# edouardoyallon/acco

Measured on AMD Instinct MI355X. Metric: tokens/s, higher is better.
Workload: dtype bf16; 1 GPU; model=llama-1b, method=acco, global_batch=8, seq_len=1024, parallelism=acco-dp1, comm_buckets=8, params=1076168704, ckpt=False

## Files before the change

acco_amd/ops/csrc/attention_bwd.hip:

```cpp

#include "attention_common.h"
#include "kernels.h"

namespace {

using namespace attn;

template <int D, int QW>
__global__ __launch_bounds__(256)
void attn_bwd_dq_kernel(const u16* __restrict__ q, const u16* __restrict__ k,
                        const u16* __restrict__ v, const u16* __restrict__ dO,
                        const float* __restrict__ lse,
                        const float* __restrict__ delta,
                        u16* __restrict__ dq,
                        int S, int H, int Hkv, float scale, int window) {
  constexpr int KS = D / 32;
  constexpr int DT = D / 16;
  constexpr int KROW = D + 8;
  constexpr int M2 = QW / 16;
  constexpr int QT = 4 * QW;
  const int qt = blockIdx.x, bh = blockIdx.y;
  const int b = bh / H, h = bh % H, hkv = h / (H / Hkv);
  const int wave = threadIdx.x >> 6, lane = threadIdx.x & 63;
  const int lg = lane >> 4, lc = lane & 15;

  extern __shared__ __attribute__((aligned(16))) u16 smem[];
  using L = BwdDqLds<D, 4>;
  u16* kT_lds = smem + L::k_t;
  u16* k_row = smem + L::k_row;
  u16* v_row = smem + L::v_row;
  u16* ds_lds = smem + L::ds + wave * 16 * LST;

  const long long qs = (long long)H * D, ks = (long long)Hkv * D;
  const int q0 = qt * QT + wave * QW;
  const u16* Qp = q + ((long long)b * S + q0) * qs + (long long)h * D;
  const u16* dOp = dO + ((long long)b * S + q0) * qs + (long long)h * D;
  const u16* Kb = k + (long long)b * S * ks + (long long)hkv * D;
  const u16* Vb = v + (long long)b * S * ks + (long long)hkv * D;

  short8 qf[M2][KS], dof[M2][KS];
  float lse_c[M2], delta_c[M2];
#pragma unroll
  for (int m = 0; m < M2; ++m) {
#pragma unroll
    for (int s = 0; s < KS; ++s) {
      qf[m][s] = *reinterpret_cast<const short8*>(
          Qp + (long long)(m * 16 + lc) * qs + s * 32 + lg * 8);
      dof[m][s] = *reinterpret_cast<const short8*>(
          dOp + (long long)(m * 16 + lc) * qs + s * 32 + lg * 8);
    }
    lse_c[m] = lse[(long long)bh * S + q0 + m * 16 + lc];
    delta_c[m] = delta[(long long)bh * S + q0 + m * 16 + lc];
  }

// ... 55 lines not shown
        for (int t = 0; t < DT; ++t) {
          short8 kb = *reinterpret_cast<const short8*>(
              kT_lds + (t * 16 + lc) * LST + s * 32 + lg * 8);
          acc_dq[m][t] = MFMA(dsa, kb, acc_dq[m][t]);
        }
      }
    }
  }

  u16* dQp = dq + ((long long)b * S + q0) * qs + (long long)h * D;
#pragma unroll
  for (int m = 0; m < M2; ++m)
#pragma unroll
    for (int r = 0; r < 4; ++r)
#pragma unroll
      for (int t = 0; t < DT; ++t)
        dQp[(long long)(m * 16 + lg * 4 + r) * qs + t * 16 + lc] =
            f32_to_bf16(acc_dq[m][t][r]);
}

template <int D, int QW>
__global__ __launch_bounds__(256)
void attn_bwd_dkv_kernel(const u16* __restrict__ q, const u16* __restrict__ k,
                         const u16* __restrict__ v, const u16* __restrict__ dO,
                         const float* __restrict__ lse,
                         const float* __restrict__ delta,
                         u16* __restrict__ dk, u16* __restrict__ dv,
                         int S, int H, int Hkv, float scale, int window) {
  constexpr int KS = D / 32;
  constexpr int DT = D / 16;
  constexpr int KROW = D + 8;
  constexpr int M2 = QW / 16;
  constexpr int KB = 4 * QW;
  const int jb = blockIdx.x, bh = blockIdx.y;
  const int b = bh / H, h = bh % H, hkv = h / (H / Hkv);
  const int wave = threadIdx.x >> 6, lane = threadIdx.x & 63;
  const int lg = lane >> 4, lc = lane & 15;

  extern __shared__ __attribute__((aligned(16))) u16 smem[];
  using L = BwdDkvLds<D, 4>;
  u16* qT_lds = smem + L::q_t;
  u16* doT_lds = smem + L::do_t;
  u16* q_row = smem + L::q_row;
  u16* do_row = smem + L::do_row;
  u16* p_lds = smem + L::p + wave * 16 * LST;
  u16* ds_lds = smem + L::p + (4 + wave) * 16 * LST;

  const long long qs = (long long)H * D, ks = (long long)Hkv * D;
  const int kv0 = jb * KB + wave * QW;
  const u16* Kp = k + ((long long)b * S + kv0) * ks + (long long)hkv * D;
  const u16* Vp = v + ((long long)b * S + kv0) * ks + (long long)hkv * D;
  const u16* Qb = q + (long long)b * S * qs + (long long)h * D;
  const u16* dOb = dO + (long long)b * S * qs + (long long)h * D;

  short8 kTf[M2][KS], vTf[M2][KS];
#pragma unroll
  for (int m = 0; m < M2; ++m)
#pragma unroll
    for (int s = 0; s < KS; ++s) {
      kTf[m][s] = *reinterpret_cast<const short8*>(
          Kp + (long long)(m * 16 + lc) * ks + s * 32 + lg * 8);
      vTf[m][s] = *reinterpret_cast<const short8*>(
          Vp + (long long)(m * 16 + lc) * ks + s * 32 + lg * 8);
    }

  f32x4 acc_dk[M2][DT] = {}, acc_dv[M2][DT] = {};

// ... 71 lines not shown
  }

  u16* dKp = dk + ((long long)b * S + kv0) * qs + (long long)h * D;
  u16* dVp = dv + ((long long)b * S + kv0) * qs + (long long)h * D;
#pragma unroll
  for (int m = 0; m < M2; ++m)
#pragma unroll
    for (int r = 0; r < 4; ++r)
#pragma unroll
      for (int t = 0; t < DT; ++t) {
        dKp[(long long)(m * 16 + lg * 4 + r) * qs + t * 16 + lc] =
            f32_to_bf16(acc_dk[m][t][r]);
        dVp[(long long)(m * 16 + lg * 4 + r) * qs + t * 16 + lc] =
            f32_to_bf16(acc_dv[m][t][r]);
      }
}

}

extern "C" {

void acco_attn_bwd_dq(const void* q, const void* k, const void* v,
                      const void* dO, const float* lse, const float* delta,
                      void* dq, int B, int S, int H, int Hkv, int D,
                      float scale, int window, hipStream_t stream) {
  if (use_mfma32(S, D)) {
    acco_attn_bwd32_dq(q, k, v, dO, lse, delta, dq, B, S, H, Hkv, D, scale,
                       window, (long long)H * D, (long long)Hkv * D,
                       (long long)H * D, (long long)H * D, nullptr, nullptr,
                       stream);
    return;
  }
  const bool w = wide(S, D);
  dim3 grid(S / (w ? 128 : 64), B * H);
#define LQ(DD, QQ) hipLaunchKernelGGL((attn_bwd_dq_kernel<DD, QQ>), grid, \
    dim3(256), (BwdDqLds<DD, 4>::bytes), stream, (const u16*)q, \
    (const u16*)k, (const u16*)v, (const u16*)dO, lse, delta, (u16*)dq, S, H, \
    Hkv, scale, window)
  if (D == 64) { if (w) LQ(64, 32); else LQ(64, 16); }
  else         LQ(128, 16);
#undef LQ
}

void acco_attn_bwd_dkv(const void* q, const void* k, const void* v,
                       const void* dO, const float* lse, const float* delta,
                       void* dk, void* dv, int B, int S, int H, int Hkv,
                       int D, float scale, int window, hipStream_t stream) {
  if (use_mfma32(S, D)) {
    acco_attn_bwd32_dkv(q, k, v, dO, lse, delta, dk, dv, B, S, H, Hkv, D,
                        scale, window, (long long)H * D, (long long)Hkv * D,
                        (long long)H * D, stream);
    return;
  }
  const bool w = wide(S, D);
  dim3 grid(S / (w ? 128 : 64), B * H);
#define LK(DD, QQ) hipLaunchKernelGGL((attn_bwd_dkv_kernel<DD, QQ>), grid, \
    dim3(256), (BwdDkvLds<DD, 4>::bytes), stream, (const u16*)q, \
    (const u16*)k, (const u16*)v, (const u16*)dO, lse, delta, (u16*)dk, \
    (u16*)dv, S, H, Hkv, scale, window)
  if (D == 64) { if (w) LK(64, 32); else LK(64, 16); }
  else         LK(128, 16);
#undef LK
}

}
```

acco_amd/ops/csrc/attention_bwd32.hip:

```cpp

#include "attention_common.h"
#include "kernels.h"

namespace {

using namespace attn;

template <int D>
__global__ __launch_bounds__(512, D == 64 ? 4 : 2)
void attn_bwd32_dq_kernel(const u16* __restrict__ q, const u16* __restrict__ k,
                          const u16* __restrict__ v, const u16* __restrict__ dO,
                          const float* __restrict__ lse,
                          const float* __restrict__ delta,
                          u16* __restrict__ dq,
                          int S, int H, int Hkv, float scale, int window,
                          long long q_rs, long long kv_rs, long long do_rs,
                          long long dq_rs,
                          const float* __restrict__ rope_cos,
                          const float* __restrict__ rope_sin) {
  constexpr int KS = D / 16;
  constexpr int DT = D / 32;
  constexpr int KROW = D + 8;
  const int qt = blockIdx.x, bh = blockIdx.y;
  const int b = bh / H, h = bh % H, hkv = h / (H / Hkv);
  const int wave = threadIdx.x >> 6, lane = threadIdx.x & 63;
  const int lq = lane & 31, hi = lane >> 5;

  extern __shared__ __attribute__((aligned(16))) u16 smem[];
  using L = Bwd32DqLds<D>;
  u16* k_row = smem + L::k_row;
  u16* v_row = smem + L::v_row;
  u16* kT_lds = smem + L::k_t;

  const long long qs = q_rs, ks = kv_rs;
  const int q0 = qt * BT32 + wave * QW32;
  const u16* Qp = q + ((long long)b * S + q0) * qs + (long long)h * D;
  const u16* dOp = dO + ((long long)b * S + q0) * do_rs + (long long)h * D;
  const u16* Kb = k + (long long)b * S * ks + (long long)hkv * D;
  const u16* Vb = v + (long long)b * S * ks + (long long)hkv * D;

  short8 qf[KS], dof[KS];
#pragma unroll
  for (int s = 0; s < KS; ++s) {
    qf[s] = *reinterpret_cast<const short8*>(
        Qp + (long long)lq * qs + s * 16 + hi * 8);
    dof[s] = *reinterpret_cast<const short8*>(
        dOp + (long long)lq * do_rs + s * 16 + hi * 8);
  }
  const float lse2_c = lse[(long long)bh * S + q0 + lq] * 1.4426950408889634f;
  const float delta_s = delta[(long long)bh * S + q0 + lq] * scale;
  const float scale2 = scale * 1.4426950408889634f;

  f32x16 acc_dq[DT] = {};

  const int j_lo = kv_tile_lo(qt * BT32, window);
  const int j_hi = kv_tile_hi(qt * BT32, BT32);
// ... 61 lines not shown
      const float* sr = rope_sin + (long long)(q0 + qrow) * D + lq;
#pragma unroll
      for (int t = 0; t < DT / 2; ++t) {
        const float c = cr[t * 32], sn = sr[t * 32];
        const float g1 = bf16_to_f32(f32_to_bf16(acc_dq[t][r]));
        const float g2 = bf16_to_f32(f32_to_bf16(acc_dq[t + DT / 2][r]));
        acc_dq[t][r] = __fmaf_rn(g1, c, __fmul_rn(g2, sn));
        acc_dq[t + DT / 2][r] = __fmaf_rn(g2, c, -__fmul_rn(g1, sn));
      }
    }
  }
#pragma unroll
  for (int r = 0; r < 16; ++r) {
    const int qrow = c32_row(r, hi);
#pragma unroll
    for (int t = 0; t < DT; ++t)
      dQp[(long long)qrow * dq_rs + t * 32 + lq] = f32_to_bf16(acc_dq[t][r]);
  }
}

template <int D>
__global__ __launch_bounds__(512)
void attn_bwd32_dkv_kernel(const u16* __restrict__ q, const u16* __restrict__ k,
                           const u16* __restrict__ v,
                           const u16* __restrict__ dO,
                           const float* __restrict__ lse,
                           const float* __restrict__ delta,
                           u16* __restrict__ dk, u16* __restrict__ dv,
                           int S, int H, int Hkv, float scale, int window,
                           long long q_rs, long long kv_rs, long long do_rs) {
  constexpr int KS = D / 16;
  constexpr int DT = D / 32;
  constexpr int KROW = D + 8;
  const int jb = blockIdx.x, bh = blockIdx.y;
  const int b = bh / H, h = bh % H, hkv = h / (H / Hkv);
  const int wave = threadIdx.x >> 6, lane = threadIdx.x & 63;
  const int lq = lane & 31, hi = lane >> 5;

  extern __shared__ __attribute__((aligned(16))) u16 smem[];
  using L = Bwd32DkvLds<D>;
  u16* q_row = smem + L::q_row;
  u16* do_row = smem + L::do_row;
  u16* qT_lds = smem + L::q_t;
  u16* doT_lds = smem + L::do_t;

  const long long qs = q_rs, ks = kv_rs;
  const long long od = (long long)H * D;
  const int kv0 = jb * BT32 + wave * QW32;
  const u16* Kp = k + ((long long)b * S + kv0) * ks + (long long)hkv * D;
  const u16* Vp = v + ((long long)b * S + kv0) * ks + (long long)hkv * D;
  const u16* Qb = q + (long long)b * S * qs + (long long)h * D;
  const u16* dOb = dO + (long long)b * S * do_rs + (long long)h * D;

  constexpr bool KV_RES = (D == 64);
  short8 kTf[KV_RES ? KS : 1], vTf[KV_RES ? KS : 1];
  if constexpr (KV_RES) {
#pragma unroll
    for (int s = 0; s < KS; ++s) {
      kTf[s] = *reinterpret_cast<const short8*>(
          Kp + (long long)lq * ks + s * 16 + hi * 8);
      vTf[s] = *reinterpret_cast<const short8*>(
          Vp + (long long)lq * ks + s * 16 + hi * 8);
    }
  }

  f32x16 acc_dk[DT] = {}, acc_dv[DT] = {};

  const int qt_lo = q_tile_lo(jb * BT32);
  const int qt_hi = q_tile_hi(jb * BT32, BT32, S, window);
  const int kv_wave_min = kv0;

  const bool t_q = (threadIdx.x < 256);
  const int t_id = threadIdx.x & 255;
  const int t_d0 = (t_id % 32) * 2;
  const int t_kv8 = (t_id / 32) * 8;
  unsigned streg[8];
  static_assert(TILE * (D / 8) % 512 == 0, "rowmajor chunks");
  constexpr int RCH = TILE * (D / 8) / 512;
  uint4 rq[RCH], rdo[RCH];

  auto load_qtile = [&](int qt) {
    const u16* Qs = Qb + (long long)(qt * TILE) * qs;
    const u16* Ds = dOb + (long long)(qt * TILE) * do_rs;
    if (D == 64) {
      const u16* Ts = t_q ? Qs : Ds;
      const long long tstride = t_q ? qs : do_rs;
#pragma unroll
      for (int r = 0; r < 8; ++r)
        streg[r] = *reinterpret_cast<const unsigned*>(
            Ts + (long long)(t_kv8 + r) * tstride + t_d0);
    }
#pragma unroll
    for (int c = 0; c < RCH; ++c) {
      const int cc = threadIdx.x + c * 512;
      const int r = cc / (D / 8), dc = cc % (D / 8);
      rq[c] = *reinterpret_cast<const uint4*>(Qs + (long long)r * qs + dc * 8);
      rdo[c] = *reinterpret_cast<const uint4*>(Ds + (long long)r * do_rs + dc * 8);
    }
  };
  auto write_qtile = [&]() {
    if (D == 64) {
      uint4 lo, hi4;
      lo.x = (streg[0] & 0xffffu) | (streg[1] << 16);
      lo.y = (streg[2] & 0xffffu) | (streg[3] << 16);
      lo.z = (streg[4] & 0xffffu) | (streg[5] << 16);
      lo.w = (streg[6] & 0xffffu) | (streg[7] << 16);
      hi4.x = (streg[0] >> 16) | (streg[1] & 0xffff0000u);
      hi4.y = (streg[2] >> 16) | (streg[3] & 0xffff0000u);
      hi4.z = (streg[4] >> 16) | (streg[5] & 0xffff0000u);
      hi4.w = (streg[6] >> 16) | (streg[7] & 0xffff0000u);
      u16* dst = t_q ? qT_lds : doT_lds;
      *reinterpret_cast<uint4*>(dst + t_d0 * LST + t_kv8) = lo;
      *reinterpret_cast<uint4*>(dst + (t_d0 + 1) * LST + t_kv8) = hi4;
    }
#pragma unroll
    for (int c = 0; c < RCH; ++c) {
      const int cc = threadIdx.x + c * 512;
      const int r = cc / (D / 8), dc = cc % (D / 8);
      reinterpret_cast<uint4*>(q_row + r * KROW)[dc] = rq[c];
      reinterpret_cast<uint4*>(do_row + r * KROW)[dc] = rdo[c];
    }
  };

  auto stage_qtile_direct = [&](int qt) {
    const u16* Qs = Qb + (long long)(qt * TILE) * qs;
    const u16* Ds = dOb + (long long)(qt * TILE) * do_rs;
    stage_transposed<D, 512>(Qs, qs, qT_lds);
    stage_transposed<D, 512>(Ds, do_rs, doT_lds);
    stage_rowmajor<D, 512>(Qs, qs, q_row);
    stage_rowmajor<D, 512>(Ds, do_rs, do_row);
  };

  if constexpr (KV_RES) load_qtile(qt_lo);
  for (int qt = qt_lo; qt <= qt_hi; ++qt) {
    __syncthreads();
    if constexpr (KV_RES) {
      write_qtile();
    } else {
      stage_qtile_direct(qt);
    }
    __syncthreads();
    if constexpr (KV_RES)
      if (qt < qt_hi) load_qtile(qt + 1);
    if (qt * TILE + TILE - 1 < kv_wave_min) continue;

#pragma unroll
    for (int m32 = 0; m32 < 2; ++m32) {
      const float lse_l =
          lse[(long long)bh * S + qt * TILE + m32 * 32 + lq] * 1.4426950408889634f;
      const float del_l =
          delta[(long long)bh * S + qt * TILE + m32 * 32 + lq] * scale;

      f32x16 st = {}, dpt = {};
      __builtin_amdgcn_s_setprio(1);
      if constexpr (KV_RES) {
#pragma unroll
        for (int s = 0; s < KS; ++s) {
          short8 qfr = *reinterpret_cast<const short8*>(
              q_row + (m32 * 32 + lq) * KROW + s * 16 + hi * 8);
          short8 dofr = *reinterpret_cast<const short8*>(
              do_row + (m32 * 32 + lq) * KROW + s * 16 + hi * 8);
          st = MFMA32(qfr, kTf[s], st);
          dpt = MFMA32(dofr, vTf[s], dpt);
        }
      } else {
#pragma unroll 2
        for (int s = 0; s < KS; ++s) {
          short8 qfr = *reinterpret_cast<const short8*>(
              q_row + (m32 * 32 + lq) * KROW + s * 16 + hi * 8);
          short8 dofr = *reinterpret_cast<const short8*>(
              do_row + (m32 * 32 + lq) * KROW + s * 16 + hi * 8);
          short8 kf = *reinterpret_cast<const short8*>(
              Kp + (long long)lq * ks + s * 16 + hi * 8);
          short8 vf = *reinterpret_cast<const short8*>(
              Vp + (long long)lq * ks + s * 16 + hi * 8);
          st = MFMA32(qfr, kf, st);
          dpt = MFMA32(dofr, vf, dpt);
        }
      }
      __builtin_amdgcn_s_setprio(0);

      const int kv_g = kv0 + lq;
      const float scale2_ = scale * 1.4426950408889634f;
      const bool need_mask =
          (qt * TILE < kv0 + QW32 - 1) ||
          (window > 0 && kv0 + window <= qt * TILE + TILE - 1);
#pragma unroll
      for (int r = 0; r < 16; ++r) {
        const int rr = c32_row(r, hi);
        const float lse_q = __shfl(lse_l, rr, 64);
        const float del_q = __shfl(del_l, rr, 64);
        float x = st[r] * scale2_ - lse_q;
        if (need_mask) {
          const int q_g = qt * TILE + m32 * 32 + rr;
          x = attends(kv_g, q_g, window) ? x : -1e30f;
        }
        const float pval = __builtin_amdgcn_exp2f(x);
        st[r] = pval;
        dpt[r] = pval * __builtin_fmaf(dpt[r], scale, -del_q);
      }

      __builtin_amdgcn_s_setprio(1);
#pragma unroll
      for (int kk = 0; kk < 2; ++kk) {
        short8 pa = c_to_afrag(st, kk);
        short8 dsa = c_to_afrag(dpt, kk);
#pragma unroll
        for (int t = 0; t < DT; ++t) {
          short8 dob = *reinterpret_cast<const short8*>(
              doT_lds + (t * 32 + lq) * LST + m32 * 32 + kk * 16 + hi * 8);
          short8 qb = *reinterpret_cast<const short8*>(
              qT_lds + (t * 32 + lq) * LST + m32 * 32 + kk * 16 + hi * 8);
          acc_dv[t] = MFMA32(pa, dob, acc_dv[t]);
          acc_dk[t] = MFMA32(dsa, qb, acc_dk[t]);
        }
      }
      __builtin_amdgcn_s_setprio(0);
    }
  }

  u16* dKp = dk + ((long long)b * S + kv0) * od + (long long)h * D;
  u16* dVp = dv + ((long long)b * S + kv0) * od + (long long)h * D;
#pragma unroll
  for (int r = 0; r < 16; ++r) {
    const int krow = c32_row(r, hi);
#pragma unroll
    for (int t = 0; t < DT; ++t) {
      dKp[(long long)krow * od + t * 32 + lq] = f32_to_bf16(acc_dk[t][r]);
      dVp[(long long)krow * od + t * 32 + lq] = f32_to_bf16(acc_dv[t][r]);
    }
  }
}

}

extern "C" {

void acco_attn_bwd32_dq(const void* q, const void* k, const void* v,
                        const void* dO, const float* lse, const float* delta,
                        void* dq, int B, int S, int H, int Hkv, int D,
                        float scale, int window, long long q_rs,
                        long long kv_rs, long long do_rs, long long dq_rs,
                        const float* rope_cos, const float* rope_sin,
                        hipStream_t stream) {
  dim3 grid(S / BT32, B * H);
#define LQ(DD) hipLaunchKernelGGL(attn_bwd32_dq_kernel<DD>, grid, dim3(512), \
    Bwd32DqLds<DD>::bytes, stream, (const u16*)q, (const u16*)k, \
    (const u16*)v, (const u16*)dO, lse, delta, (u16*)dq, S, H, Hkv, scale, \
    window, q_rs, kv_rs, do_rs, dq_rs, rope_cos, rope_sin)
  if (D == 64) LQ(64); else LQ(128);
#undef LQ
}

void acco_attn_bwd32_dkv(const void* q, const void* k, const void* v,
                         const void* dO, const float* lse,
                         const float* delta, void* dk, void* dv, int B,
                         int S, int H, int Hkv, int D, float scale,
                         int window, long long q_rs, long long kv_rs,
                         long long do_rs, hipStream_t stream) {
  dim3 grid(S / BT32, B * H);
#define LK(DD) hipLaunchKernelGGL(attn_bwd32_dkv_kernel<DD>, grid, dim3(512), \
    Bwd32DkvLds<DD>::bytes, stream, (const u16*)q, (const u16*)k, \
    (const u16*)v, (const u16*)dO, lse, delta, (u16*)dk, (u16*)dv, S, H, Hkv, \
    scale, window, q_rs, kv_rs, do_rs)
  if (D == 64) LK(64); else LK(128);
#undef LK
}

}
```

acco_amd/ops/csrc/attention_common.h:

```cpp
#pragma once

#include "common.h"

namespace attn {

using u16 = unsigned short;
using short8 = __attribute__((ext_vector_type(8))) short;
using f32x4 = __attribute__((ext_vector_type(4))) float;
using f32x16 = __attribute__((ext_vector_type(16))) float;

constexpr int TILE = 64;
constexpr int PAD = 8;
constexpr int LST = TILE + PAD;
constexpr int QW32 = 32, NW32 = 8, BT32 = QW32 * NW32;

#define MFMA(a, b, c) \
  __builtin_amdgcn_mfma_f32_16x16x32_bf16((a), (b), (c), 0, 0, 0)
#define MFMA32(a, b, c) \
  __builtin_amdgcn_mfma_f32_32x32x16_bf16((a), (b), (c), 0, 0, 0)


template <int D, int NT>
ACCO_DEV void stage_transposed(const u16* src, long long row_stride,
                               u16* dst) {
// ... 49 lines not shown
  reinterpret_cast<unsigned*>(&pa)[2] = r02[1];
  reinterpret_cast<unsigned*>(&pa)[3] = r13[1];
  return pa;
}

ACCO_DEV int kv_tile_lo(int q_blk0, int window) {
  int j_lo = 0;
  if (window > 0) {
    int kv_min = q_blk0 - window + 1;
    if (kv_min > 0) j_lo = kv_min / TILE;
  }
  return j_lo;
}
ACCO_DEV int kv_tile_hi(int q_blk0, int rows) {
  return (q_blk0 + rows - 1) / TILE;
}

ACCO_DEV int q_tile_lo(int kv_blk0) { return kv_blk0 / TILE; }
ACCO_DEV int q_tile_hi(int kv_blk0, int rows, int S, int window) {
  int qt_hi = S / TILE - 1;
  if (window > 0) {
    const int q_lim = kv_blk0 + rows - 1 + window;
    qt_hi = min(qt_hi, q_lim / TILE);
  }
  return qt_hi;
}

ACCO_DEV bool attends(int kv_g, int q_g, int window) {
  bool valid = (kv_g <= q_g);
  if (window > 0) valid = valid && (kv_g > q_g - window);
  return valid;
}

constexpr int t_tile(int D) { return D * LST; }
constexpr int r_tile(int D) { return TILE * (D + 8); }
constexpr int w_tile(int NW) { return NW * 16 * LST; }

template <int D, int NW> struct FwdLds {
  static constexpr int v_t = 0, k_row = v_t + t_tile(D),
                       p = k_row + r_tile(D),
                       bytes = (p + w_tile(NW)) * sizeof(u16);
};
template <int D> struct Fwd32Lds {
  static constexpr int k_row = 0, v_t = k_row + r_tile(D),
                       bytes = (v_t + t_tile(D)) * sizeof(u16);
};
template <int D, int NW> struct BwdDqLds {
  static constexpr int k_t = 0, k_row = k_t + t_tile(D),
                       v_row = k_row + r_tile(D),
                       ds = v_row + r_tile(D),
                       bytes = (ds + w_tile(NW)) * sizeof(u16);
};
template <int D, int NW> struct BwdDkvLds {
  static constexpr int q_t = 0, do_t = q_t + t_tile(D),
                       q_row = do_t + t_tile(D), do_row = q_row + r_tile(D),
                       p = do_row + r_tile(D),
                       bytes = (p + 2 * w_tile(NW)) * sizeof(u16);
};
template <int D> struct Bwd32DqLds {
  static constexpr int k_row = 0, v_row = k_row + r_tile(D),
                       k_t = v_row + r_tile(D),
                       bytes = (k_t + t_tile(D)) * sizeof(u16);
};
template <int D> struct Bwd32DkvLds {
  static constexpr int q_row = 0, do_row = q_row + r_tile(D),
                       q_t = do_row + r_tile(D), do_t = q_t + t_tile(D),
                       bytes = (do_t + t_tile(D)) * sizeof(u16);
};

inline bool use_mfma32(int S, int D) {
  return (D == 64 || D == 128) && S % BT32 == 0;
}
inline bool wide(int S, int D) { return (S % 128 == 0) && (D == 64); }

}
```

acco_amd/ops/csrc/attention_fwd.hip:

```cpp

#include "attention_common.h"
#include "kernels.h"

namespace {

using namespace attn;

template <int D, int QW>
__global__ __launch_bounds__(256)
void attn_fwd_kernel(const u16* __restrict__ q, const u16* __restrict__ k,
                     const u16* __restrict__ v, u16* __restrict__ o,
                     float* __restrict__ lse,
                     int S, int H, int Hkv, float scale, int window) {
  constexpr int KS = D / 32;
  constexpr int DT = D / 16;
  constexpr int M2 = QW / 16;
  constexpr int QT = 4 * QW;
  constexpr int KROW = D + 8;
  const int qt = blockIdx.x;
  const int bh = blockIdx.y;
  const int b = bh / H, h = bh % H;
  const int hkv = h / (H / Hkv);
  const int wave = threadIdx.x >> 6;
  const int lane = threadIdx.x & 63;
  const int lg = lane >> 4;
  const int lc = lane & 15;

  using L = FwdLds<D, 4>;
  extern __shared__ __attribute__((aligned(16))) u16 smem[];
  u16* v_lds = smem + L::v_t;
  u16* k_lds = smem + L::k_row;
  u16* p_lds = smem + L::p + wave * 16 * LST;

  const int q0 = qt * QT + wave * QW;
  const long long qs = (long long)H * D;
  const long long ks = (long long)Hkv * D;
  const u16* Qp = q + ((long long)b * S + q0) * qs + (long long)h * D;
  const u16* Kb = k + (long long)b * S * ks + (long long)hkv * D;
  const u16* Vb = v + (long long)b * S * ks + (long long)hkv * D;

  short8 qf[M2][KS];
#pragma unroll
  for (int m = 0; m < M2; ++m)
#pragma unroll
    for (int s = 0; s < KS; ++s)
      qf[m][s] = *reinterpret_cast<const short8*>(
          Qp + (long long)(m * 16 + lc) * qs + s * 32 + lg * 8);

  float m_c[M2], l_c[M2] = {};
  f32x4 acc_o[M2][DT] = {};
#pragma unroll
  for (int m = 0; m < M2; ++m) m_c[m] = -1e30f;

// ... 94 lines not shown
#pragma unroll
  for (int m = 0; m < M2; ++m) {
    float l_row[4];
#pragma unroll
    for (int r = 0; r < 4; ++r)
      l_row[r] = __shfl(l_c[m], lg * 4 + r, 64);
#pragma unroll
    for (int r = 0; r < 4; ++r) {
      const float inv_l = (l_row[r] > 0.f) ? 1.0f / l_row[r] : 0.0f;
#pragma unroll
      for (int t = 0; t < DT; ++t)
        Op[(long long)(m * 16 + lg * 4 + r) * qs + t * 16 + lc] =
            f32_to_bf16(acc_o[m][t][r] * inv_l);
    }
    if (lg == 0)
      lse[((long long)bh) * S + q0 + m * 16 + lc] =
          m_c[m] + __logf(fmaxf(l_c[m], 1e-30f));
  }
}

}

extern "C" void acco_attn_fwd(const void* q, const void* k, const void* v,
                              void* o, float* lse, int B, int S, int H,
                              int Hkv, int D, float scale, int window,
                              hipStream_t stream) {
  if (use_mfma32(S, D)) {
    acco_attn_fwd32(q, k, v, o, lse, B, S, H, Hkv, D, scale, window,
                    (long long)H * D, (long long)Hkv * D, (long long)H * D,
                    stream);
    return;
  }
  const bool w = wide(S, D);
  dim3 grid(S / (w ? 128 : 64), B * H);
#define LA(DD, QQ) hipLaunchKernelGGL((attn_fwd_kernel<DD, QQ>), grid, \
    dim3(256), (FwdLds<DD, 4>::bytes), stream, (const u16*)q, (const u16*)k, \
    (const u16*)v, (u16*)o, lse, S, H, Hkv, scale, window)
  if (D == 64) { if (w) LA(64, 32); else LA(64, 16); }
  else         LA(128, 16);
#undef LA
}
```

acco_amd/ops/csrc/attention_fwd32.hip:

```cpp

#include "attention_common.h"
#include "kernels.h"

namespace {

using namespace attn;

template <int D>
__global__ __launch_bounds__(512, D == 64 ? 4 : 2)
void attn_fwd32_kernel(const u16* __restrict__ q, const u16* __restrict__ k,
                       const u16* __restrict__ v, u16* __restrict__ o,
                       float* __restrict__ lse,
                       int S, int H, int Hkv, float scale, int window,
                       long long q_rs, long long kv_rs, long long o_rs) {
  constexpr int KS = D / 16;
  constexpr int DT = D / 32;
  const int qt = blockIdx.x;
  const int bh = blockIdx.y;
  const int b = bh / H, h = bh % H;
  const int hkv = h / (H / Hkv);
  const int wave = threadIdx.x >> 6;
  const int lane = threadIdx.x & 63;
  const int lq = lane & 31;
  const int hi = lane >> 5;

  extern __shared__ __attribute__((aligned(16))) u16 smem[];
  u16* k_lds = smem + Fwd32Lds<D>::k_row;
  u16* v_lds = smem + Fwd32Lds<D>::v_t;
  constexpr int KROW = D + 8;

  const int q0 = qt * BT32 + wave * QW32;
  const long long qs = q_rs;
  const long long ks = kv_rs;
  const u16* Qp = q + ((long long)b * S + q0) * qs + (long long)h * D;
  const u16* Kb = k + (long long)b * S * ks + (long long)hkv * D;
  const u16* Vb = v + (long long)b * S * ks + (long long)hkv * D;

  short8 qf[KS];
#pragma unroll
  for (int s = 0; s < KS; ++s)
    qf[s] = *reinterpret_cast<const short8*>(
        Qp + (long long)lq * qs + s * 16 + hi * 8);

  float m_c = -1e30f, l_c = 0.0f;
  f32x16 acc_o[DT] = {};

  const int j_lo = kv_tile_lo(qt * BT32, window);
  const int j_hi = kv_tile_hi(qt * BT32, BT32);
  const int q_wave_max = q0 + QW32 - 1;
  const float scale2 = scale * 1.4426950408889634f;
  constexpr float THR2 = 8.0f * 1.4426950408889634f;
// ... 82 lines not shown
        }
      }
    }
    __builtin_amdgcn_s_setprio(0);
  }

  float l_row[16];
#pragma unroll
  for (int r = 0; r < 16; ++r)
    l_row[r] = __shfl(l_c, c32_row(r, hi), 64);
  u16* Op = o + ((long long)b * S + q0) * o_rs + (long long)h * D;
#pragma unroll
  for (int r = 0; r < 16; ++r) {
    const float inv_l = (l_row[r] > 0.f) ? 1.0f / l_row[r] : 0.0f;
    const int qrow = c32_row(r, hi);
#pragma unroll
    for (int t = 0; t < DT; ++t)
      Op[(long long)qrow * o_rs + t * 32 + lq] =
          f32_to_bf16(acc_o[t][r] * inv_l);
  }
  if (hi == 0)
    lse[((long long)bh) * S + q0 + lq] =
        (m_c + __builtin_amdgcn_logf(fmaxf(l_c, 1e-30f))) *
        0.6931471805599453f;
}

}

extern "C" void acco_attn_fwd32(const void* q, const void* k, const void* v,
                                void* o, float* lse, int B, int S, int H,
                                int Hkv, int D, float scale, int window,
                                long long q_rs, long long kv_rs,
                                long long o_rs, hipStream_t stream) {
  dim3 grid(S / BT32, B * H);
#define LA(DD) hipLaunchKernelGGL(attn_fwd32_kernel<DD>, grid, dim3(512), \
    Fwd32Lds<DD>::bytes, stream, (const u16*)q, (const u16*)k, \
    (const u16*)v, (u16*)o, lse, S, H, Hkv, scale, window, q_rs, kv_rs, o_rs)
  if (D == 64) LA(64); else LA(128);
#undef LA
}
```

acco_amd/ops/csrc/bindings.cpp:

```cpp
#include <torch/extension.h>
#include <ATen/hip/HIPContext.h>
#include <c10/hip/HIPException.h>

#include <hip/hip_runtime.h>

#include "kernels.h"

namespace {

using u16 = unsigned short;

void fused_adamw(at::Tensor p, at::Tensor g, at::Tensor m, at::Tensor v,
                 int64_t step, double lr, double beta1, double beta2,
                 double eps, double weight_decay, double scale,
                 at::Tensor scale_dev, at::Tensor out, bool commit) {
  TORCH_CHECK(p.is_cuda() && p.scalar_type() == at::kFloat && p.is_contiguous());
  TORCH_CHECK(m.sizes() == p.sizes() && v.sizes() == p.sizes());
  TORCH_CHECK(g.numel() == p.numel() && g.is_contiguous());
  const bool bf16 = g.scalar_type() == at::kBFloat16;
  TORCH_CHECK(bf16 || g.scalar_type() == at::kFloat,
              "grad must be bf16 or fp32");
  void* out_ptr = nullptr;
  if (out.numel() > 0) {
    TORCH_CHECK(out.numel() == p.numel() && out.is_contiguous());
// ... 283 lines not shown
              lse.data_ptr<float>(), dlogits.data_ptr(),
              acc.data_ptr<float>(), (float)dloss, nullptr, T, S, V,
              (float)epsilon, cur_stream());
  return dlogits;
}

at::Tensor ce_bwd_dev(at::Tensor logits, at::Tensor labels, at::Tensor lse,
                      at::Tensor acc, at::Tensor dloss_dev, double epsilon) {
  CHECK_BF16_CONTIG(logits);
  TORCH_CHECK(dloss_dev.is_cuda() && dloss_dev.scalar_type() == at::kFloat &&
              dloss_dev.numel() == 1);
  const long long Bn = logits.size(0);
  const int S = (int)logits.size(1), V = (int)logits.size(2);
  const long long T = Bn * S;
  auto dlogits = at::empty_like(logits);
  acco_ce_bwd(logits.data_ptr(),
              reinterpret_cast<const long long*>(labels.data_ptr<int64_t>()),
              lse.data_ptr<float>(), dlogits.data_ptr(),
              acc.data_ptr<float>(), 0.0f, dloss_dev.data_ptr<float>(), T, S,
              V, (float)epsilon, cur_stream());
  return dlogits;
}

struct AttnShape { int B, S, H, Hkv, D; };

static AttnShape check_attn_dims(int64_t B, int64_t S, int64_t H, int64_t Hkv,
                                 int64_t D, int64_t window, int64_t s_mult) {
  TORCH_CHECK((D == 64 || D == 128) && H > 0 && Hkv > 0 && H % Hkv == 0,
              "need D in {64, 128} and H % Hkv == 0, got D=", D, " H=", H,
              " Hkv=", Hkv);
  TORCH_CHECK(S > 0 && S % s_mult == 0 && S < (1LL << 30) && window >= 0,
              "need S % ", s_mult, " == 0 and window >= 0, got S=", S,
              " window=", window);
  TORCH_CHECK(B > 0 && B * H <= 65535, "need 1 <= B*H <= 65535 (grid.y), got ",
              "B=", B, " H=", H);
  return {(int)B, (int)S, (int)H, (int)Hkv, (int)D};
}

static void check_attn_like(const at::Tensor& ref, const char* what,
                            std::initializer_list<at::Tensor> same) {
  for (const at::Tensor& t : same) {
    CHECK_BF16_CONTIG(t);
    TORCH_CHECK(t.device() == ref.device() && t.sizes() == ref.sizes(), what,
                ": expected ", ref.sizes(), " on ", ref.device(), ", got ",
                t.sizes(), " on ", t.device());
  }
}

static void check_attn_stats(const at::Tensor& ref, const AttnShape& a,
                             std::initializer_list<at::Tensor> stats) {
  const int64_t n = (int64_t)a.B * a.H * a.S;
  for (const at::Tensor& st : stats)
    TORCH_CHECK(st.is_cuda() && st.device() == ref.device() &&
                st.scalar_type() == at::kFloat && st.is_contiguous() &&
                st.numel() == n, "lse/delta must be contiguous CUDA fp32 with "
                "B*H*S = ", n, " elements, got ", st.numel(), " of ",
                st.scalar_type());
}

static AttnShape check_attn_args(
    const at::Tensor& q, const at::Tensor& k, const at::Tensor& v,
    int64_t window, std::initializer_list<at::Tensor> like_q = {},
    std::initializer_list<at::Tensor> stats = {}) {
  CHECK_BF16_CONTIG(q); CHECK_BF16_CONTIG(k);
  TORCH_CHECK(q.dim() == 4 && k.dim() == 4 && k.device() == q.device() &&
              k.size(0) == q.size(0) && k.size(1) == q.size(1) &&
              k.size(3) == q.size(3),
              "need q [B,S,H,D] and k [B,S,Hkv,D] on one device, got ",
// ... 23 lines not shown
  CHECK_BF16_CONTIG(dO);
  TORCH_CHECK(dO.dim() == 4 && dO.size(3) % 8 == 0 && dO.size(1) < (1LL << 31),
              "dO must be [B,S,H,D] with D % 8 == 0, got ", dO.sizes());
  check_attn_like(dO, "o against dO", {o});
  const long long B = dO.size(0);
  const int S = (int)dO.size(1), H = (int)dO.size(2), D = (int)dO.size(3);
  auto delta = at::empty({B, H, S}, dO.options().dtype(at::kFloat));
  acco_attn_delta(dO.data_ptr(), o.data_ptr(), delta.data_ptr<float>(), B, S,
                  H, D, cur_stream());
  C10_HIP_KERNEL_LAUNCH_CHECK();
  return delta;
}

std::vector<at::Tensor> attn_bwd(at::Tensor q, at::Tensor k, at::Tensor v,
                                 at::Tensor dO, at::Tensor lse,
                                 at::Tensor delta, double scale,
                                 int64_t window) {
  const auto [B, S, H, Hkv, D] =
      check_attn_args(q, k, v, window, {dO}, {lse, delta});
  auto dq = at::empty_like(q);
  auto dk = at::empty_like(q);
  auto dv = at::empty_like(q);
  acco_attn_bwd_dq(q.data_ptr(), k.data_ptr(), v.data_ptr(), dO.data_ptr(),
                   lse.data_ptr<float>(), delta.data_ptr<float>(),
                   dq.data_ptr(), B, S, H, Hkv, D, (float)scale, (int)window,
                   cur_stream());
  C10_HIP_KERNEL_LAUNCH_CHECK();
  acco_attn_bwd_dkv(q.data_ptr(), k.data_ptr(), v.data_ptr(), dO.data_ptr(),
                    lse.data_ptr<float>(), delta.data_ptr<float>(),
                    dk.data_ptr(), dv.data_ptr(), B, S, H, Hkv, D,
                    (float)scale, (int)window, cur_stream());
  C10_HIP_KERNEL_LAUNCH_CHECK();
  return {dq, dk, dv};
}

struct PackedSection { const char* name; int64_t off, width; };

static void check_packed_layout(const at::Tensor& qkv,
                                std::initializer_list<PackedSection> secs) {
  CHECK_BF16_CONTIG(qkv);
  TORCH_CHECK(qkv.dim() == 3 && qkv.size(2) % 8 == 0,
              "packed qkv must be [B,S,W] with W % 8 == 0, got ", qkv.sizes());
  const int64_t W = qkv.size(2);
  for (const PackedSection& s : secs) {
    TORCH_CHECK(s.off >= 0 && s.off % 8 == 0 && s.width > 0 &&
                s.off + s.width <= W, s.name, " section [", s.off, ", ",
                s.off + s.width, ") must start at a multiple of 8 inside W=",
                W);
    for (const PackedSection& t : secs)
      TORCH_CHECK(&s == &t || s.off + s.width <= t.off ||
                  t.off + t.width <= s.off, s.name, " section [", s.off, ", ",
                  s.off + s.width, ") overlaps ", t.name, " section [", t.off,
                  ", ", t.off + t.width, ")");
  }
}

static void gqa_reduce_impl(const at::Tensor& dkq, const at::Tensor& dvq,
                            const at::Tensor& dqkv, const at::Tensor* cos_t,
                            const at::Tensor* sin_t, int64_t Hkv, int64_t rep,
                            int64_t D, int64_t k_off, int64_t v_off) {
  CHECK_BF16_CONTIG(dkq);
  TORCH_CHECK(Hkv > 0 && rep > 0 && D > 0 && D % (cos_t ? 16 : 8) == 0 &&
              dkq.dim() == 4 && dkq.size(2) == Hkv * rep && dkq.size(3) == D,
              "dkq/dvq must be [B, S, Hkv*rep, D] with D % ", cos_t ? 16 : 8,
              " == 0, got ", dkq.sizes(), " for Hkv=", Hkv, " rep=", rep,
              " D=", D);
// ... 152 lines not shown

PYBIND11_MODULE(TORCH_EXTENSION_NAME, m) {
  m.def("fused_adamw", &fused_adamw,
        "Fused sharded AdamW (gfx950): cast+scale+AdamW+bf16 writeout; "
        "commit=false = ACCO tentative step");
  m.def("swiglu_fwd", &swiglu_fwd);
  m.def("swiglu_bwd", &swiglu_bwd);
  m.def("swiglu_packed_fwd", &swiglu_packed_fwd);
  m.def("swiglu_packed_bwd", &swiglu_packed_bwd);
  m.def("gelu_fwd", &gelu_fwd);
  m.def("gelu_bwd", &gelu_bwd);
  m.def("colsum", &colsum);
  m.def("rmsnorm_fwd", &rmsnorm_fwd);
  m.def("rmsnorm_bwd", &rmsnorm_bwd, py::arg("dy"), py::arg("x"),
        py::arg("w"), py::arg("rstd"), py::arg("dadd") = py::none());
  m.def("add_rmsnorm_fwd", &add_rmsnorm_fwd);
  m.def("layernorm_fwd", &layernorm_fwd);
  m.def("layernorm_bwd", &layernorm_bwd, py::arg("dy"), py::arg("x"),
        py::arg("w"), py::arg("mean"), py::arg("rstd"),
        py::arg("dadd") = py::none());
  m.def("add_layernorm_fwd", &add_layernorm_fwd);
  m.def("rope_fwd", &rope_fwd);
  m.def("ce_fwd", &ce_fwd, py::arg("logits"), py::arg("labels"),
        py::arg("epsilon") = 0.0);
  m.def("ce_bwd", &ce_bwd, py::arg("logits"), py::arg("labels"),
        py::arg("lse"), py::arg("acc"), py::arg("dloss"),
        py::arg("epsilon") = 0.0);
  m.def("ce_bwd_dev", &ce_bwd_dev, py::arg("logits"), py::arg("labels"),
        py::arg("lse"), py::arg("acc"), py::arg("dloss_dev"),
        py::arg("epsilon") = 0.0);
  m.def("attn_fwd", &attn_fwd);
  m.def("attn_delta", &attn_delta);
  m.def("attn_bwd", &attn_bwd);
  m.def("attn_gqa_reduce", &attn_gqa_reduce);
  m.def("attn_gqa_reduce_rope", &attn_gqa_reduce_rope);
  m.def("rope_qk_inplace", &rope_qk_inplace);
  m.def("gemm_nt", &gemm_nt);
  m.def("rope_packed", &rope_packed);
  m.def("attn_fwd_packed", &attn_fwd_packed);
  m.def("attn_bwd_packed", &attn_bwd_packed, py::arg("qkv"), py::arg("dO"),
        py::arg("lse"), py::arg("delta"), py::arg("dqkv"), py::arg("H"),
        py::arg("Hkv"), py::arg("D"), py::arg("scale"), py::arg("window"),
        py::arg("q_off"), py::arg("k_off"), py::arg("v_off"),
        py::arg("cos") = py::none(), py::arg("sin") = py::none());
  m.attr("_gfx950") = true;
}
```

acco_amd/ops/csrc/kernels.h:

```cpp
#pragma once

#include <hip/hip_runtime.h>

extern "C" {

void acco_fused_adamw_launch(void* p, const void* g, void* m, void* v,
                             void* out, const float* scale_dev, long long n,
                             bool buf_is_bf16, bool commit, float scale,
                             float lr, float beta1, float beta2, float eps,
                             float weight_decay, long long step_plus_1,
                             hipStream_t stream);

void acco_swiglu_fwd(const void* g, const void* u, void* out, long long n,
                     int cols, long long row_stride8, hipStream_t s);
void acco_swiglu_bwd(const void* dout, const void* g, const void* u, void* dg,
                     void* du, long long n, int cols, long long row_stride8,
                     hipStream_t s);
void acco_gelu_fwd(const void* x, void* out, long long n, hipStream_t s);
void acco_gelu_bwd(const void* dout, const void* x, void* dx, long long n,
                   hipStream_t s);

void acco_rmsnorm_fwd(const void* x, const void* w, void* y, void* rstd,
                      const void* res, void* sum_out, long long R, int D,
                      float eps, hipStream_t s);
// ... 12 lines not shown
void acco_norm_dw_finalize(const float* dw_part, const float* db_part,
                           void* dw, void* db, int P, int D, bool out_bf16,
                           hipStream_t s);
void acco_colsum(const void* in, float* out, long long P, int D,
                 bool in_is_bf16, hipStream_t s);

void acco_rope(const void* x, void* y, const float* cos_t, const float* sin_t,
               long long B, int S, int H, int D, bool bwd,
               long long row_stride, hipStream_t stream);
void acco_rope_qk_inplace(void* qkv, const float* cos_t, const float* sin_t,
                          long long T, int S, int H, int Hkv, int D,
                          long long W, long long q_off, long long k_off,
                          hipStream_t stream);

void acco_ce_fwd(const void* logits, const long long* labels, float* lse,
                 float* acc, long long T, int S, int V, float epsilon,
                 hipStream_t s);
void acco_ce_bwd(const void* logits, const long long* labels,
                 const float* lse, void* dlogits, const float* acc,
                 float dloss, const float* dloss_dev, long long T, int S,
                 int V, float epsilon, hipStream_t s);

void acco_gemm_nt(const void* A, const void* B, void* C, int M, int N, int K,
                  hipStream_t stream);

void acco_attn_fwd(const void* q, const void* k, const void* v, void* o,
                   float* lse, int B, int S, int H, int Hkv, int D,
                   float scale, int window, hipStream_t stream);
void acco_attn_fwd32(const void* q, const void* k, const void* v, void* o,
                     float* lse, int B, int S, int H, int Hkv, int D,
                     float scale, int window, long long q_rs, long long kv_rs,
                     long long o_rs, hipStream_t stream);

void acco_attn_bwd_dq(const void* q, const void* k, const void* v,
                      const void* dO, const float* lse, const float* delta,
                      void* dq, int B, int S, int H, int Hkv, int D,
                      float scale, int window, hipStream_t stream);
void acco_attn_bwd_dkv(const void* q, const void* k, const void* v,
                       const void* dO, const float* lse, const float* delta,
                       void* dk, void* dv, int B, int S, int H, int Hkv,
                       int D, float scale, int window, hipStream_t stream);
void acco_attn_bwd32_dq(const void* q, const void* k, const void* v,
                        const void* dO, const float* lse, const float* delta,
                        void* dq, int B, int S, int H, int Hkv, int D,
                        float scale, int window, long long q_rs,
                        long long kv_rs, long long do_rs, long long dq_rs,
                        const float* rope_cos, const float* rope_sin,
                        hipStream_t stream);
void acco_attn_bwd32_dkv(const void* q, const void* k, const void* v,
                         const void* dO, const float* lse,
                         const float* delta, void* dk, void* dv, int B,
                         int S, int H, int Hkv, int D, float scale,
                         int window, long long q_rs, long long kv_rs,
                         long long do_rs, hipStream_t stream);

void acco_attn_delta(const void* dO, const void* O, float* delta, long long B,
                     int S, int H, int D, hipStream_t stream);
void acco_attn_gqa_reduce(const void* dkq, const void* dvq, void* dqkv,
                          long long T, int Hkv, int rep, int D, long long W,
                          long long k_off, long long v_off,
                          hipStream_t stream);
void acco_attn_gqa_reduce_rope(const void* dkq, const void* dvq, void* dqkv,
                               const float* cos_t, const float* sin_t,
                               long long T, int S, int Hkv, int rep, int D,
                               long long W, long long k_off, long long v_off,
                               hipStream_t stream);
// ... 3 lines not shown
```

Measured before the change: 122,500 tokens/s.

## Schedule causal attention blocks heavy-first via 1-D grid and stage LSE/delta in LDS

```diff
diff --git a/acco_amd/ops/csrc/attention_bwd.hip b/acco_amd/ops/csrc/attention_bwd.hip
--- a/acco_amd/ops/csrc/attention_bwd.hip
+++ b/acco_amd/ops/csrc/attention_bwd.hip
@@ -19,7 +19,9 @@
   constexpr int KROW = D + 8;
   constexpr int M2 = QW / 16;
   constexpr int QT = 4 * QW;
-  const int qt = blockIdx.x, bh = blockIdx.y;
+  const BlockPos pos = block_order(
+      blockIdx.x, S / QT, gridDim.x / (S / QT), true);
+  const int qt = pos.row_block, bh = pos.bh;
   const int b = bh / H, h = bh % H, hkv = h / (H / Hkv);
   const int wave = threadIdx.x >> 6, lane = threadIdx.x & 63;
   const int lg = lane >> 4, lc = lane & 15;
@@ -141,7 +143,9 @@
   constexpr int KROW = D + 8;
   constexpr int M2 = QW / 16;
   constexpr int KB = 4 * QW;
-  const int jb = blockIdx.x, bh = blockIdx.y;
+  const BlockPos pos = block_order(
+      blockIdx.x, S / KB, gridDim.x / (S / KB), false);
+  const int jb = pos.row_block, bh = pos.bh;
   const int b = bh / H, h = bh % H, hkv = h / (H / Hkv);
   const int wave = threadIdx.x >> 6, lane = threadIdx.x & 63;
   const int lg = lane >> 4, lc = lane & 15;
@@ -279,7 +283,7 @@
     return;
   }
   const bool w = wide(S, D);
-  dim3 grid(S / (w ? 128 : 64), B * H);
+  dim3 grid(block_order_grid(S / (w ? 128 : 64), B, H));
 #define LQ(DD, QQ) hipLaunchKernelGGL((attn_bwd_dq_kernel<DD, QQ>), grid, \
     dim3(256), (BwdDqLds<DD, 4>::bytes), stream, (const u16*)q, \
     (const u16*)k, (const u16*)v, (const u16*)dO, lse, delta, (u16*)dq, S, H, \
@@ -300,7 +304,7 @@
     return;
   }
   const bool w = wide(S, D);
-  dim3 grid(S / (w ? 128 : 64), B * H);
+  dim3 grid(block_order_grid(S / (w ? 128 : 64), B, H));
 #define LK(DD, QQ) hipLaunchKernelGGL((attn_bwd_dkv_kernel<DD, QQ>), grid, \
     dim3(256), (BwdDkvLds<DD, 4>::bytes), stream, (const u16*)q, \
     (const u16*)k, (const u16*)v, (const u16*)dO, lse, delta, (u16*)dk, \
diff --git a/acco_amd/ops/csrc/attention_bwd32.hip b/acco_amd/ops/csrc/attention_bwd32.hip
--- a/acco_amd/ops/csrc/attention_bwd32.hip
+++ b/acco_amd/ops/csrc/attention_bwd32.hip
@@ -21,7 +21,9 @@
   constexpr int KS = D / 16;
   constexpr int DT = D / 32;
   constexpr int KROW = D + 8;
-  const int qt = blockIdx.x, bh = blockIdx.y;
+  const BlockPos pos = block_order(
+      blockIdx.x, S / BT32, gridDim.x / (S / BT32), true);
+  const int qt = pos.row_block, bh = pos.bh;
   const int b = bh / H, h = bh % H, hkv = h / (H / Hkv);
   const int wave = threadIdx.x >> 6, lane = threadIdx.x & 63;
   const int lq = lane & 31, hi = lane >> 5;
@@ -149,7 +151,9 @@
   constexpr int KS = D / 16;
   constexpr int DT = D / 32;
   constexpr int KROW = D + 8;
-  const int jb = blockIdx.x, bh = blockIdx.y;
+  const BlockPos pos = block_order(
+      blockIdx.x, S / BT32, gridDim.x / (S / BT32), false);
+  const int jb = pos.row_block, bh = pos.bh;
   const int b = bh / H, h = bh % H, hkv = h / (H / Hkv);
   const int wave = threadIdx.x >> 6, lane = threadIdx.x & 63;
   const int lq = lane & 31, hi = lane >> 5;
@@ -160,6 +164,7 @@
   u16* do_row = smem + L::do_row;
   u16* qT_lds = smem + L::q_t;
   u16* doT_lds = smem + L::do_t;
+  float* stat_lds = reinterpret_cast<float*>(smem + L::stats);
 
   const long long qs = q_rs, ks = kv_rs;
   const long long od = (long long)H * D;
@@ -195,10 +200,16 @@
   static_assert(TILE * (D / 8) % 512 == 0, "rowmajor chunks");
   constexpr int RCH = TILE * (D / 8) / 512;
   uint4 rq[RCH], rdo[RCH];
+  const bool st_on = (threadIdx.x < 2 * TILE);
+  const float* st_src = (threadIdx.x < TILE ? lse : delta) +
+                        (long long)bh * S + (threadIdx.x & (TILE - 1));
+  const float st_mul = (threadIdx.x < TILE) ? 1.4426950408889634f : scale;
+  float streg_stat = 0.0f;
 
   auto load_qtile = [&](int qt) {
     const u16* Qs = Qb + (long long)(qt * TILE) * qs;
     const u16* Ds = dOb + (long long)(qt * TILE) * do_rs;
+    if (st_on) streg_stat = st_src[qt * TILE];
     if (D == 64) {
       const u16* Ts = t_q ? Qs : Ds;
       const long long tstride = t_q ? qs : do_rs;
@@ -216,6 +227,7 @@
     }
   };
   auto write_qtile = [&]() {
+    if (st_on) stat_lds[threadIdx.x] = streg_stat * st_mul;
     if (D == 64) {
       uint4 lo, hi4;
       lo.x = (streg[0] & 0xffffu) | (streg[1] << 16);
@@ -246,6 +258,7 @@
     stage_transposed<D, 512>(Ds, do_rs, doT_lds);
     stage_rowmajor<D, 512>(Qs, qs, q_row);
     stage_rowmajor<D, 512>(Ds, do_rs, do_row);
+    if (st_on) stat_lds[threadIdx.x] = st_src[qt * TILE] * st_mul;
   };
 
   if constexpr (KV_RES) load_qtile(qt_lo);
@@ -263,11 +276,6 @@
 
 #pragma unroll
     for (int m32 = 0; m32 < 2; ++m32) {
-      const float lse_l =
-          lse[(long long)bh * S + qt * TILE + m32 * 32 + lq] * 1.4426950408889634f;
-      const float del_l =
-          delta[(long long)bh * S + qt * TILE + m32 * 32 + lq] * scale;
-
       f32x16 st = {}, dpt = {};
       __builtin_amdgcn_s_setprio(1);
       if constexpr (KV_RES) {
@@ -302,11 +310,15 @@
       const bool need_mask =
           (qt * TILE < kv0 + QW32 - 1) ||
           (window > 0 && kv0 + window <= qt * TILE + TILE - 1);
+      const float* lse_r = stat_lds + m32 * 32 + 4 * hi;
+      const float* del_r = lse_r + TILE;
 #pragma unroll
       for (int r = 0; r < 16; ++r) {
         const int rr = c32_row(r, hi);
-        const float lse_q = __shfl(lse_l, rr, 64);
-        const float del_q = __shfl(del_l, rr, 64);
+        const float lse_q =
+            (*reinterpret_cast<const f32x4*>(lse_r + 8 * (r >> 2)))[r & 3];
+        const float del_q =
+            (*reinterpret_cast<const f32x4*>(del_r + 8 * (r >> 2)))[r & 3];
         float x = st[r] * scale2_ - lse_q;
         if (need_mask) {
           const int q_g = qt * TILE + m32 * 32 + rr;
@@ -360,7 +372,7 @@
                         long long kv_rs, long long do_rs, long long dq_rs,
                         const float* rope_cos, const float* rope_sin,
                         hipStream_t stream) {
-  dim3 grid(S / BT32, B * H);
+  dim3 grid(block_order_grid(S / BT32, B, H));
 #define LQ(DD) hipLaunchKernelGGL(attn_bwd32_dq_kernel<DD>, grid, dim3(512), \
     Bwd32DqLds<DD>::bytes, stream, (const u16*)q, (const u16*)k, \
     (const u16*)v, (const u16*)dO, lse, delta, (u16*)dq, S, H, Hkv, scale, \
@@ -375,7 +387,7 @@
                          int S, int H, int Hkv, int D, float scale,
                          int window, long long q_rs, long long kv_rs,
                          long long do_rs, hipStream_t stream) {
-  dim3 grid(S / BT32, B * H);
+  dim3 grid(block_order_grid(S / BT32, B, H));
 #define LK(DD) hipLaunchKernelGGL(attn_bwd32_dkv_kernel<DD>, grid, dim3(512), \
     Bwd32DkvLds<DD>::bytes, stream, (const u16*)q, (const u16*)k, \
     (const u16*)v, (const u16*)dO, lse, delta, (u16*)dk, (u16*)dv, S, H, Hkv, \
diff --git a/acco_amd/ops/csrc/attention_common.h b/acco_amd/ops/csrc/attention_common.h
--- a/acco_amd/ops/csrc/attention_common.h
+++ b/acco_amd/ops/csrc/attention_common.h
@@ -105,6 +105,19 @@
   return valid;
 }
 
+struct BlockPos { int row_block, bh; };
+
+__host__ __device__ __forceinline__ BlockPos block_order(
+    unsigned id, unsigned n_blk, unsigned BH, bool heavy_last) {
+  const unsigned level = id / BH;
+  return {(int)(heavy_last ? n_blk - 1 - level : level),
+          (int)(id - level * BH)};
+}
+
+inline unsigned block_order_grid(int n_blk, int B, int H) {
+  return (unsigned)n_blk * (unsigned)(B * H);
+}
+
 constexpr int t_tile(int D) { return D * LST; }
 constexpr int r_tile(int D) { return TILE * (D + 8); }
 constexpr int w_tile(int NW) { return NW * 16 * LST; }
@@ -138,7 +151,9 @@
 template <int D> struct Bwd32DkvLds {
   static constexpr int q_row = 0, do_row = q_row + r_tile(D),
                        q_t = do_row + r_tile(D), do_t = q_t + t_tile(D),
-                       bytes = (do_t + t_tile(D)) * sizeof(u16);
+                       stats = do_t + t_tile(D),
+                       bytes = stats * sizeof(u16) + 2 * TILE * sizeof(float);
+  static_assert(stats * sizeof(u16) % 16 == 0, "stats rows are read as float4");
 };
 
 inline bool use_mfma32(int S, int D) {
diff --git a/acco_amd/ops/csrc/attention_fwd.hip b/acco_amd/ops/csrc/attention_fwd.hip
--- a/acco_amd/ops/csrc/attention_fwd.hip
+++ b/acco_amd/ops/csrc/attention_fwd.hip
@@ -17,8 +17,9 @@
   constexpr int M2 = QW / 16;
   constexpr int QT = 4 * QW;
   constexpr int KROW = D + 8;
-  const int qt = blockIdx.x;
-  const int bh = blockIdx.y;
+  const BlockPos pos = block_order(
+      blockIdx.x, S / QT, gridDim.x / (S / QT), true);
+  const int qt = pos.row_block, bh = pos.bh;
   const int b = bh / H, h = bh % H;
   const int hkv = h / (H / Hkv);
   const int wave = threadIdx.x >> 6;
@@ -179,7 +180,7 @@
     return;
   }
   const bool w = wide(S, D);
-  dim3 grid(S / (w ? 128 : 64), B * H);
+  dim3 grid(block_order_grid(S / (w ? 128 : 64), B, H));
 #define LA(DD, QQ) hipLaunchKernelGGL((attn_fwd_kernel<DD, QQ>), grid, \
     dim3(256), (FwdLds<DD, 4>::bytes), stream, (const u16*)q, (const u16*)k, \
     (const u16*)v, (u16*)o, lse, S, H, Hkv, scale, window)
@@ -187,3 +188,13 @@
   else         LA(128, 16);
 #undef LA
 }
+
+extern "C" void acco_attn_block_order(int* out, int n_blk, int B, int H,
+                                      bool heavy_last) {
+  const unsigned n = block_order_grid(n_blk, B, H);
+  for (unsigned id = 0; id < n; ++id) {
+    const BlockPos pos = block_order(id, n_blk, B * H, heavy_last);
+    out[2 * id] = pos.row_block;
+    out[2 * id + 1] = pos.bh;
+  }
+}
diff --git a/acco_amd/ops/csrc/attention_fwd32.hip b/acco_amd/ops/csrc/attention_fwd32.hip
--- a/acco_amd/ops/csrc/attention_fwd32.hip
+++ b/acco_amd/ops/csrc/attention_fwd32.hip
@@ -15,8 +15,9 @@
                        long long q_rs, long long kv_rs, long long o_rs) {
   constexpr int KS = D / 16;
   constexpr int DT = D / 32;
-  const int qt = blockIdx.x;
-  const int bh = blockIdx.y;
+  const BlockPos pos = block_order(
+      blockIdx.x, S / BT32, gridDim.x / (S / BT32), true);
+  const int qt = pos.row_block, bh = pos.bh;
   const int b = bh / H, h = bh % H;
   const int hkv = h / (H / Hkv);
   const int wave = threadIdx.x >> 6;
@@ -165,7 +166,7 @@
                                 int Hkv, int D, float scale, int window,
                                 long long q_rs, long long kv_rs,
                                 long long o_rs, hipStream_t stream) {
-  dim3 grid(S / BT32, B * H);
+  dim3 grid(block_order_grid(S / BT32, B, H));
 #define LA(DD) hipLaunchKernelGGL(attn_fwd32_kernel<DD>, grid, dim3(512), \
     Fwd32Lds<DD>::bytes, stream, (const u16*)q, (const u16*)k, \
     (const u16*)v, (u16*)o, lse, S, H, Hkv, scale, window, q_rs, kv_rs, o_rs)
diff --git a/acco_amd/ops/csrc/bindings.cpp b/acco_amd/ops/csrc/bindings.cpp
--- a/acco_amd/ops/csrc/bindings.cpp
+++ b/acco_amd/ops/csrc/bindings.cpp
@@ -339,8 +339,9 @@
   TORCH_CHECK(S > 0 && S % s_mult == 0 && S < (1LL << 30) && window >= 0,
               "need S % ", s_mult, " == 0 and window >= 0, got S=", S,
               " window=", window);
-  TORCH_CHECK(B > 0 && B * H <= 65535, "need 1 <= B*H <= 65535 (grid.y), got ",
-              "B=", B, " H=", H);
+  TORCH_CHECK(B > 0 && B * H <= 65535 && (S / 64) * B * H < (1LL << 31),
+              "need 1 <= B*H <= 65535 and S/64 * B*H < 2^31 (the 1-D grid), "
+              "got B=", B, " H=", H, " S=", S);
   return {(int)B, (int)S, (int)H, (int)Hkv, (int)D};
 }
 
@@ -430,6 +431,18 @@
                     (float)scale, (int)window, cur_stream());
   C10_HIP_KERNEL_LAUNCH_CHECK();
   return {dq, dk, dv};
+}
+
+at::Tensor attn_block_order(int64_t n_blk, int64_t B, int64_t H,
+                            bool heavy_last) {
+  TORCH_CHECK(B > 0 && H > 0 && B * H <= 65535 && n_blk > 0 &&
+              n_blk < (1LL << 31) && n_blk * B * H < (1LL << 31),
+              "need 1 <= B*H <= 65535 and 1 <= n_blk*B*H < 2^31, got n_blk=",
+              n_blk, " B=", B, " H=", H);
+  auto out = at::empty({n_blk * B * H, 2}, at::TensorOptions().dtype(at::kInt));
+  acco_attn_block_order(out.data_ptr<int>(), (int)n_blk, (int)B, (int)H,
+                        heavy_last);
+  return out;
 }
 
 struct PackedSection { const char* name; int64_t off, width; };
@@ -648,6 +661,8 @@
   m.def("attn_fwd", &attn_fwd);
   m.def("attn_delta", &attn_delta);
   m.def("attn_bwd", &attn_bwd);
+  m.def("attn_block_order", &attn_block_order, py::arg("n_blk"),
+        py::arg("B"), py::arg("H"), py::arg("heavy_last"));
   m.def("attn_gqa_reduce", &attn_gqa_reduce);
   m.def("attn_gqa_reduce_rope", &attn_gqa_reduce_rope);
   m.def("rope_qk_inplace", &rope_qk_inplace);
diff --git a/acco_amd/ops/csrc/kernels.h b/acco_amd/ops/csrc/kernels.h
--- a/acco_amd/ops/csrc/kernels.h
+++ b/acco_amd/ops/csrc/kernels.h
@@ -68,6 +68,9 @@
                      float scale, int window, long long q_rs, long long kv_rs,
                      long long o_rs, hipStream_t stream);
 
+void acco_attn_block_order(int* out, int n_blk, int B, int H,
+                           bool heavy_last);
+
 void acco_attn_bwd_dq(const void* q, const void* k, const void* v,
                       const void* dO, const float* lse, const float* delta,
                       void* dq, int B, int S, int H, int Hkv, int D,
```

Result: faster. 128,500 tokens/s (median of 6 runs) (+4.9%).
